# GenomicBreeding/GenomicBreedingModels.jl

Hardware: AMD Instinct MI355X
Metric: GRM+GBLUP genotype-cells/s (n x p) (higher is better)
Workload: dtype f64

## Files before the change

### genomicbreedingmodels.jl_amd/csrc/gbm_internal.h

```cpp
#pragma once
#include <hip/hip_runtime.h>
#include <stdint.h>
#include <functional>
#include <string>
#include <vector>

#include "../../include/gbm.h"

namespace gbm {

constexpr int64_t kNPadTile = 128;
constexpr int64_t kRhsRows = 64;
constexpr int kCholNB = 64;

inline int64_t round_up(int64_t x, int64_t m) { return (x + m - 1) / m * m; }
inline int64_t npad_of(int64_t n) { return round_up(n < 1 ? 1 : n, kNPadTile); }
inline int64_t gdim_of(int64_t n) { return npad_of(n) + kRhsRows; }

void set_error(const std::string& msg);
int fail(int code, const std::string& msg);
const std::string& last_error();

const char* knob(const char* name);
int64_t knob_i64(const char* name, int64_t def);

#define GBM_HIP_TRY(expr)                                                                      \
  do {                                                                                         \
    hipError_t e_ = (expr);                                                                    \
    if (e_ != hipSuccess)                                                                      \
      return ::gbm::fail(GBM_E_HIP, std::string("HIP error '") + hipGetErrorString(e_) +       \
                                        "' at " __FILE__ ":" + std::to_string(__LINE__) + " (" #expr ")"); \
  } while (0)

#define GBM_LAUNCH_CHECK() GBM_HIP_TRY(hipGetLastError())

#define GBM_TRY(expr)              \
  do {                             \
    int rc_ = (expr);              \
    if (rc_ != GBM_OK) return rc_; \
  } while (0)

int launch_grm(const double* Zt, int64_t ldz, int64_t p, int64_t n, double* G, int64_t ldg,
               void* ws, int64_t ws_bytes, hipStream_t s, int accum = 0, int32_t* err_out = nullptr);
bool grm_can_accumulate(int64_t n, int64_t p);
int64_t grm_workspace_bytes(int64_t n, int64_t p);
int launch_grm_export(const double* G, int64_t ldg, int64_t n, double inv_q, double* out, int64_t ldo, hipStream_t s);
int launch_predict(const double* Xt, int64_t ldx, int64_t p, int64_t n, const double* b, int64_t ldb, int64_t nrhs,
                   double* partial, int64_t nchunks, double* out, int64_t ldo, hipStream_t s);
int64_t predict_chunks(int64_t n, int64_t p);
int launch_add_inplace(double* a, const double* b, int64_t n, hipStream_t s);
int launch_standardize_i8(const int8_t* D, int64_t ldd, int64_t p, int64_t n, int ploidy, double* Zt, int64_t ldz,
                          double* mean, double* sd, int32_t* keep, int64_t* q_dev, hipStream_t s);
int launch_marker_rows(const double* Zt, int64_t ldz, int64_t p, int64_t n, const double* A, int64_t lda, int64_t nrhs,
                       double inv_q, const int64_t* q_dev, const double* sd, const int32_t* keep, double* B,
                       int64_t ldb, hipStream_t s);
int launch_marker_rows_i8(const int8_t* D, int64_t ldd, int64_t p, int64_t n, int ploidy, const double* A, int64_t lda,
                          int64_t nrhs, double inv_q, const int64_t* q_dev, const double* mean, const double* sd,
                          const int32_t* keep, double* B, int64_t ldb, hipStream_t s);
int launch_grm_exact(const int8_t* D, int64_t ldd, int64_t p, int64_t n, int ploidy, double* G, int64_t ldg,
                     double* mean, double* sd, int32_t* keep, int64_t* q_dev, int accum, void* ws, int64_t ws_bytes,
                     int32_t* slices_out, hipStream_t s);
int grm_exact_status(const void* ws, int64_t n, int64_t p, hipStream_t s);
int launch_gather_dosage(const double* Xt, int64_t ldx, int64_t p, const int32_t* idx, int64_t nT, int8_t* D,
                         hipStream_t s);
int launch_dosage_from_f64(const double* X, int64_t ldx, int64_t n, int64_t p, int8_t* D, int64_t ldd, int32_t* bad,
                           hipStream_t s);
int launch_dosage_check_i8(const int8_t* D, int64_t ldd, int64_t n, int64_t p, int32_t* bad, hipStream_t s);
// ... 58 lines not shown
```

### genomicbreedingmodels.jl_amd/csrc/grm.hip

```cpp
#include <algorithm>
#include <atomic>
#include <cmath>
#include <cstdio>
#include <cstdlib>
#include <map>
#include <mutex>
#include <queue>
#include <tuple>
#include <vector>

#include "chol_device.h"

namespace gbm {

constexpr int BT = 128;
constexpr int BK = 16;
constexpr int WPS = 2;
constexpr int LROW = BT + 2;
constexpr int STAGE = 2 * BK * LROW;

__device__ __forceinline__ void tile_of(int64_t t, int64_t& ti, int64_t& tj) {
  int64_t r = (int64_t)((sqrt(8.0 * (double)t + 1.0) - 1.0) * 0.5);
  while ((r + 1) * (r + 2) / 2 <= t) r++;
  while (r * (r + 1) / 2 > t) r--;
// ... 148 lines not shown

__device__ __forceinline__ void diag_tile(const double* __restrict__ U, int64_t ldu, int64_t K, int64_t i0,
                                          int64_t kstep0, int64_t nsteps, double* lds, double* __restrict__ out,
                                          int64_t ld, int wave, int lane) {
  asm volatile("" : "+v"(lane));
  switch (wave) {
    case 0: diag_tile_wave<0>(U, ldu, K, i0, kstep0, nsteps, lds, out, ld, lane); break;
    case 1: diag_tile_wave<1>(U, ldu, K, i0, kstep0, nsteps, lds, out, ld, lane); break;
    case 2: diag_tile_wave<2>(U, ldu, K, i0, kstep0, nsteps, lds, out, ld, lane); break;
    default: diag_tile_wave<3>(U, ldu, K, i0, kstep0, nsteps, lds, out, ld, lane); break;
  }
}

constexpr int kMaxSlices = 32;
struct SliceBounds {
  int32_t n;
  int32_t b[kMaxSlices + 1];
  int32_t carry;
  int32_t er, et, erb, es, ekper;
  int64_t e0, eslab_off;
  int32_t accum = 0;
  int32_t fuse = 0;
  int32_t diag = 0;
};

template <int ET>
__device__ __forceinline__ void grm_edge_pass(const double* __restrict__ U, int64_t ldu, int64_t K,
                                              const SliceBounds& sb, int64_t e, double* __restrict__ part,
                                              int lane, int wave) {
  const int rb = (int)(e % sb.erb), ks = (int)(e / sb.erb);
  const int64_t k0 = (int64_t)ks * sb.ekper;
  const int64_t k1 = (k0 + sb.ekper < K) ? k0 + sb.ekper : K;
  const int64_t i0 = (int64_t)rb * 256 + wave * 64;
  const int fr = lane >> 4, fc = lane & 15;
  d4 acc[4][ET];
#pragma unroll
  for (int m = 0; m < 4; m++)
#pragma unroll
    for (int q = 0; q < ET; q++) acc[m][q] = (d4){0.0, 0.0, 0.0, 0.0};
  for (int64_t k = k0; k < k1; k += 16) {
    double a[4][4], b[4][ET];
#pragma unroll
    for (int st = 0; st < 4; st++) {
      const int64_t kk = k + st * 4 + fr;
      const bool kv = kk < k1;
      const double* row = U + kk * ldu;
// ... 189 lines not shown
#pragma unroll
        for (int r = 0; r < 4; r++) {
          double* o = out + (16 * r + m) * ld;
          *reinterpret_cast<double2*>(o) = make_double2(acc[m][0][r], acc[m][1][r]);
          *reinterpret_cast<double2*>(o + 2) = make_double2(acc[m][2][r], acc[m][3][r]);
        }
    }
    };
    const int64_t T8 = (ntiles + 7) & ~(int64_t)7;
    if constexpr (MODE == kPersist || MODE == kPersistFused) {
      __shared__ int64_t s_unit;
      int32_t* ctr = info;
      const int xcc = (int)(__builtin_amdgcn_s_getreg((20 << 0) | (0 << 6) | (31 << 11)) & 7);
      const int64_t per = T8 >> 3;
      int q = xcc;
      for (int tries = 0; tries < 8;) {
        const int64_t qt0 = q * per;
        const int64_t qt1 = qt0 + per < ntiles ? qt0 + per : ntiles;
        const int64_t nq = qt1 > qt0 ? qt1 - qt0 : 0;
        if (threadIdx.x == 0) s_unit = atomicAdd(&ctr[q], 1);
        __syncthreads();
        const int64_t u = s_unit;
        __syncthreads();
        if (u >= nq * sb.n) {
          q = (q + 1) & 7;
          tries++;
          continue;
        }
        const int sl = (int)(u / nq);
        run_unit(sl, qt0 + (u - (int64_t)sl * nq));
      }
      return;
    } else {
      const int sl = (int)(wg / T8);
      const int64_t u = wg - (int64_t)sl * T8;
      const int64_t t = (u & 7) * (T8 >> 3) + (u >> 3);
      if (t >= ntiles) return;
      run_unit(sl, t);
    }
    return;
  } else {
    int64_t ti, tj;
    if (own.nranks > 1) {
      const int64_t c = blockIdx.y;
      const int64_t J = c < own.ncols ? own.j_first + c * own.nranks : own.rhs_tile;
      tj = J - c0 / BT;
      ti = own.ti0 + blockIdx.x;
      if (ti > tj) return;
    } else {
      tile_of(wg, ti, tj);
    }
    const bool diag = (ti == tj);
    const int64_t i0 = c0 + ti * BT, j0 = c0 + tj * BT;
// ... 464 lines not shown
  GBM_HIP_TRY(hipGetDevice(&dev));
  if (caller) {
    int sdev = -1;
    if (hipStreamGetDevice(caller, &sdev) != hipSuccess) {
      (void)hipGetLastError();
      return GBM_OK;
    }
    if (sdev != dev) return GBM_OK;
  }
  static std::mutex mu;
  static std::map<int, hipStream_t> streams;
  {
    std::lock_guard<std::mutex> lock(mu);
    hipStream_t& hs = streams[dev];
    if (!hs) GBM_HIP_TRY(hipStreamCreateWithFlags(&hs, hipStreamNonBlocking));
    a.s = hs;
  }
  GBM_HIP_TRY(hipEventCreateWithFlags(&a.fork, hipEventDisableTiming));
  GBM_HIP_TRY(hipEventCreateWithFlags(&a.join, hipEventDisableTiming));
  *usable = true;
  return GBM_OK;
}

static int64_t grm_counter_doubles(const GrmPlan& g) { return 4 + (g.sb.fuse ? (g.ntiles + 1) / 2 : 0); }
int64_t grm_workspace_bytes(int64_t n, int64_t p) {
  const GrmPlan g = plan(n, p);
  return (g.main_doubles + g.edge_doubles + grm_counter_doubles(g)) * (int64_t)sizeof(double);
}

static int check_grm_args(const double* Zt, int64_t ldz, int64_t p, int64_t n, double* G, int64_t ldg) {
  const int64_t npad = npad_of(n);
  if (!Zt || !G || p < 1 || n < 1 || ldz < npad || ldg < npad || (ldz & 1) || (ldg & 1))
    return fail(GBM_E_ARG, "gbm_dev_grm: bad arguments (need ldz, ldg >= npad(n), both even)");
  if (((uintptr_t)Zt & 15) != 0 || ((uintptr_t)G & 15) != 0)
    return fail(GBM_E_ARG, "gbm_dev_grm: Zt and G must be 16-byte aligned");
  return GBM_OK;
}

int launch_grm_syrk(const double* Zt, int64_t ldz, int64_t p, int64_t n, double* G, int64_t ldg, void* ws,
                    int64_t ws_bytes, hipStream_t s, int accum = 0) {
  int rc = check_grm_args(Zt, ldz, p, n, G, ldg);
  if (rc != GBM_OK) return rc;
  const GrmPlan g = plan(n, p);
  SliceBounds sb = g.sb;
  sb.accum = accum;
  const int64_t need = (g.main_doubles + g.edge_doubles + grm_counter_doubles(g)) * (int64_t)sizeof(double);
  if (need > 0 && (!ws || ws_bytes < need))
    return fail(GBM_E_ARG, "gbm_dev_grm: workspace too small (" + std::to_string(ws_bytes) + " < " +
                               std::to_string(need) + ")");
  const unsigned grid = (unsigned)(g.sb.n * ((g.ntiles + 7) & ~(int64_t)7));
  if (g.sb.carry) GBM_HIP_TRY(hipMemsetAsync(ws, 0, (size_t)(g.ntiles + 1) * sizeof(int32_t), s));
  int32_t* ctr = reinterpret_cast<int32_t*>((double*)ws + g.main_doubles + g.edge_doubles);
  const int64_t lim = g.sb.er > 0 ? g.sb.e0 : n;
  AuxStream aux;
  AuxStream* ax = nullptr;
  if (g.edge_concurrent) {
    bool usable = false;
    rc = aux_stream(s, aux, &usable);
    if (rc != GBM_OK) return rc;
    if (usable) {
      ax = &aux;
      GBM_HIP_TRY(hipEventRecord(ax->fork, s));
      GBM_HIP_TRY(hipStreamWaitEvent(ax->s, ax->fork, 0));
    }
  }
  if (g.persist) {
    GBM_HIP_TRY(hipMemsetAsync(ctr, 0, (size_t)(8 + (g.sb.fuse ? g.ntiles : 0)) * sizeof(int32_t), s));
    const int64_t units = (int64_t)g.sb.n * g.ntiles;
    const unsigned pgrid = (unsigned)(units < resident_wgs() ? units : resident_wgs());
    if (g.sb.fuse)
      syrk_kernel<kPersistFused><<<pgrid, 256, 0, s>>>(Zt, ldz, p, 0, lim, G, ldg, (double*)ws, g.ntiles, sb, nullptr,
                                                       nullptr, ctr, -1, TileOwner{});
    else
      syrk_kernel<kPersist><<<pgrid, 256, 0, s>>>(Zt, ldz, p, 0, lim, G, ldg, (double*)ws, g.ntiles, sb, nullptr,
                                                  nullptr, ctr, -1, TileOwner{});
  } else {
    syrk_kernel<kSplit><<<grid, 256, 0, s>>>(Zt, ldz, p, 0, lim, G, ldg, (double*)ws, g.ntiles, sb, nullptr, nullptr,
                                             nullptr, -1, TileOwner{});
  }
  GBM_LAUNCH_CHECK();
  if (g.sb.er > 0) {
    const hipStream_t es = ax ? ax->s : s;
    const unsigned eg = (unsigned)((int64_t)g.sb.erb * g.sb.es);
    double* part = (double*)ws + g.sb.eslab_off;
    switch (g.sb.et) {
      case 1: grm_edge_kernel<1><<<eg, 256, 0, es>>>(Zt, ldz, p, g.sb, part); break;
      case 2: grm_edge_kernel<2><<<eg, 256, 0, es>>>(Zt, ldz, p, g.sb, part); break;
      case 3: grm_edge_kernel<3><<<eg, 256, 0, es>>>(Zt, ldz, p, g.sb, part); break;
      default: grm_edge_kernel<4><<<eg, 256, 0, es>>>(Zt, ldz, p, g.sb, part); break;
    }
    GBM_LAUNCH_CHECK();
    if (g.edge_concurrent) {
      grm_edge_reduce_kernel<<<(unsigned)((n * g.sb.er + 255) / 256), 256, 0, es>>>(part, n, g.sb, G, ldg, accum);
      GBM_LAUNCH_CHECK();
    }
    if (ax) {
      GBM_HIP_TRY(hipEventRecord(ax->join, ax->s));
      GBM_HIP_TRY(hipStreamWaitEvent(s, ax->join, 0));
    }
  }
  return GBM_OK;
}

int launch_grm_reduce(int64_t n, int64_t p, double* G, int64_t ldg, const void* ws, hipStream_t s, int accum = 0,
                      int32_t* err_out = nullptr) {
  const GrmPlan g = plan(n, p);
  if (g.sb.n == 1 && g.sb.er == 0) return GBM_OK;
  if (!ws) return fail(GBM_E_ARG, "gbm_dev_grm_reduce: workspace required");
  if (g.sb.er > 0 && !g.edge_concurrent) {
    grm_edge_reduce_kernel<<<(unsigned)((n * g.sb.er + 255) / 256), 256, 0, s>>>((const double*)ws + g.sb.eslab_off, n,
                                                                                 g.sb, G, ldg, accum);
    GBM_LAUNCH_CHECK();
  }
  if (g.sb.n == 1 || g.sb.fuse) return GBM_OK;
  if (g.sb.carry && err_out) {
    GBM_HIP_TRY(hipMemcpyAsync(err_out, (const int32_t*)ws + g.ntiles, sizeof(int32_t), hipMemcpyDeviceToDevice, s));
    return GBM_OK;
  }
  if (g.sb.carry) {
    int32_t err = 0;
    GBM_HIP_TRY(hipMemcpyAsync(&err, (const int32_t*)ws + g.ntiles, sizeof(int32_t), hipMemcpyDeviceToHost, s));
    GBM_HIP_TRY(hipStreamSynchronize(s));
    if (err < 0)
// ... 59 lines not shown
  return GBM_OK;
}

extern "C" int64_t gbm_dev_grm_workspace(int64_t n, int64_t p) { return gbm::grm_workspace_bytes(n, p); }

extern "C" int gbm_dev_grm(const double* Zt, int64_t ldz, int64_t p, int64_t n, double* G, int64_t ldg,
                           void* workspace, int64_t ws_bytes, void* stream) {
  return gbm::launch_grm(Zt, ldz, p, n, G, ldg, workspace, ws_bytes, (hipStream_t)stream);
}

extern "C" int gbm_dev_grm_accumulate(const double* Zt, int64_t ldz, int64_t p, int64_t n, double* G, int64_t ldg,
                                      void* workspace, int64_t ws_bytes, void* stream) {
  if (!gbm::grm_can_accumulate(n, p))
    return gbm::fail(GBM_E_ARG, "gbm_dev_grm_accumulate: this (n, p) plans a single loci range (gbm_dev_grm_slices == 1); "
                                "use more loci per call");
  return gbm::launch_grm(Zt, ldz, p, n, G, ldg, workspace, ws_bytes, (hipStream_t)stream, 1);
}

extern "C" int gbm_dev_grm_syrk(const double* Zt, int64_t ldz, int64_t p, int64_t n, double* G, int64_t ldg,
                                void* workspace, int64_t ws_bytes, void* stream) {
  return gbm::launch_grm_syrk(Zt, ldz, p, n, G, ldg, workspace, ws_bytes, (hipStream_t)stream);
}

extern "C" int gbm_dev_grm_reduce(int64_t n, int64_t p, double* G, int64_t ldg, const void* workspace, void* stream) {
  if (!G || n < 1 || p < 1 || ldg < gbm::npad_of(n)) return gbm::fail(GBM_E_ARG, "gbm_dev_grm_reduce: bad arguments");
  return gbm::launch_grm_reduce(n, p, G, ldg, workspace, (hipStream_t)stream);
}

extern "C" int gbm_dev_grm_slices(int64_t n, int64_t p) {
  return gbm::plan(n, p).sb.n;
}

namespace gbm {
__global__ void __launch_bounds__(256) add_inplace_kernel(double* __restrict__ a, const double* __restrict__ b,
                                                          int64_t n) {
  for (int64_t i = ((int64_t)blockIdx.x * 256 + threadIdx.x) * 2; i < n; i += (int64_t)gridDim.x * 512) {
    if (i + 1 < n) {
      double2 x = *reinterpret_cast<const double2*>(a + i);
      const double2 y = *reinterpret_cast<const double2*>(b + i);
      x.x += y.x;
      x.y += y.y;
      *reinterpret_cast<double2*>(a + i) = x;
    } else {
      a[i] += b[i];
    }
  }
// ... 24 lines not shown
```

### genomicbreedingmodels.jl_amd/csrc/stats.hip

```cpp
#include <type_traits>

#include "gbm_internal.h"

namespace gbm {

__device__ __forceinline__ uint64_t mix64(uint64_t z) {
  z += 0x9E3779B97F4A7C15ull;
  z = (z ^ (z >> 30)) * 0xBF58476D1CE4E5B9ull;
  z = (z ^ (z >> 27)) * 0x94D049BB133111EBull;
  return z ^ (z >> 31);
}

__global__ void __launch_bounds__(256) synth_kernel(double* __restrict__ Xt, int64_t ldx, int64_t p,
                                                    int64_t n, uint64_t seed, int64_t j0) {
  for (int64_t j = blockIdx.y; j < p; j += gridDim.y) {
    const uint64_t base = mix64(seed * 0xD1B54A32D192ED03ull + (uint64_t)(j0 + j));
    const uint64_t thr = 214748364ull + (((base >> 32) * 1932735283ull) >> 32);
    double* row = Xt + j * ldx;
    for (int64_t i = (int64_t)blockIdx.x * 1024 + threadIdx.x; i < (int64_t)(blockIdx.x + 1) * 1024 && i < ldx;
         i += 256) {
      double v = 0.0;
      if (i < n) {
        const uint64_t h = mix64(base ^ ((uint64_t)i * 0x8CB92BA72F3D8DD7ull));
        const int d = ((h & 0xFFFFFFFFull) < thr) + ((h >> 32) < thr);
// ... 251 lines not shown
    else if (n <= 64 * 64) GBM_STD_W(64);
    else if (n <= 64 * 80) GBM_STD_W(80);
    else if (n <= 64 * 96) GBM_STD_W(96);
    else GBM_STD_W(128);
#undef GBM_STD_W
    GBM_LAUNCH_CHECK();
    return GBM_OK;
  }
  if (n <= 256 * 4)
    standardize_kernel<256, 4, GATHER, T><<<grid, 256, 0, s>>>(Xt, ldx, p, idx, n, Zt, ldz, mean, sd, keep, q, center_only, xs);
  else if (n <= 256 * 8)
    standardize_kernel<256, 8, GATHER, T><<<grid, 256, 0, s>>>(Xt, ldx, p, idx, n, Zt, ldz, mean, sd, keep, q, center_only, xs);
  else if (n <= 256 * 16)
    standardize_kernel<256, 16, GATHER, T><<<grid, 256, 0, s>>>(Xt, ldx, p, idx, n, Zt, ldz, mean, sd, keep, q, center_only, xs);
  else if (n <= 256 * 32)
    standardize_kernel<256, 32, GATHER, T><<<grid, 256, 0, s>>>(Xt, ldx, p, idx, n, Zt, ldz, mean, sd, keep, q, center_only, xs);
  else
    standardize_kernel<256, 0, GATHER, T><<<grid, 256, 0, s>>>(Xt, ldx, p, idx, n, Zt, ldz, mean, sd, keep, q, center_only, xs);
  GBM_LAUNCH_CHECK();
  return GBM_OK;
}

namespace gbm {
int launch_center_columns(const double* Xt, int64_t ldx, int64_t p, int64_t n, double* Zt, int64_t ldz, double* mean,
                          double* sd, int32_t* keep, int64_t* q_dev, hipStream_t s) {
  if (p == 0) return GBM_OK;
  return launch_standardize<false>(Xt, ldx, p, nullptr, n, Zt, ldz, mean, sd, keep, q_dev, 1, s);
}

int launch_standardize_i8(const int8_t* D, int64_t ldd, int64_t p, int64_t n, int ploidy, double* Zt, int64_t ldz,
                          double* mean, double* sd, int32_t* keep, int64_t* q_dev, hipStream_t s) {
  if (!D || !Zt || !mean || !sd || !keep || !q_dev || p < 0 || n < 1 || ldd < n || ldz < n || ploidy < 1)
    return fail(GBM_E_ARG, "standardize (int8 dosages): bad arguments");
  if (p == 0) return GBM_OK;
  return launch_standardize<false, int8_t>(D, ldd, p, nullptr, n, Zt, ldz, mean, sd, keep, q_dev, 0, s, 1.0 / ploidy);
}
}

extern "C" int gbm_dev_standardize(const double* Xt, int64_t ldx, int64_t p, int64_t n, double* Zt, int64_t ldz,
                                   double* mean, double* sd, int32_t* keep, int64_t* q_dev, void* stream) {
  if (!Xt || !Zt || !mean || !sd || !keep || !q_dev || p < 0 || n < 1 || ldx < n || ldz < n ||
      ((const double*)Zt == Xt && ldz != ldx))
    return fail(GBM_E_ARG, "gbm_dev_standardize: bad arguments");
  if (p == 0) return GBM_OK;
  return launch_standardize<false>(Xt, ldx, p, nullptr, n, Zt, ldz, mean, sd, keep, q_dev, 0, (hipStream_t)stream);
}
// ... 18 lines not shown
```

### genomicbreedingmodels.jl_amd/gbm/_lib.py

```python
from __future__ import annotations

import ctypes
import os
import threading

import numpy as np

ABI_VERSION = 212
GBM_OK = 0
GBM_E_ARG = -1
GBM_E_NOTPD = -2
GBM_E_HIP = -3
GBM_E_RCCL = -4
GBM_E_OOM = -5
GBM_E_NODEV = -6
GBM_E_DATA = -7

LIB_PATH = os.environ.get("GBM_LIBGBM") or os.path.join(os.path.dirname(os.path.abspath(__file__)), "libgbm.so")

EXPORTS = (
    "gbm_version", "gbm_last_error", "gbm_device_count", "gbm_device_allocations", "gbm_release_device_cache",
    "gbm_gblup_fit", "gbm_gblup_fit_reml", "gbm_gblup_fit_dosage_i8", "gbm_gblup_fit_synthetic", "gbm_grm", "gbm_grm_ploidy_aware", "gbm_colstats", "gbm_predict",
    "gbm_dev_npad", "gbm_dev_gdim", "gbm_dev_grm_workspace", "gbm_dev_solve_workspace",
    "gbm_dev_synth_genotypes", "gbm_dev_expand_dosage_i8", "gbm_dev_standardize", "gbm_dev_grm",
    "gbm_dev_grm_syrk", "gbm_dev_grm_reduce", "gbm_dev_grm_slices",
    "gbm_dev_gblup_solve", "gbm_dev_marker_effects",
    "gbm_dev_standardize_gather", "gbm_dev_gblup_terms",
    "gbm_session_create", "gbm_session_create_dosage_i8", "gbm_session_create_synthetic", "gbm_session_destroy", "gbm_session_gblup_fit",
    "gbm_session_predict", "gbm_session_reml_objective", "gbm_session_reml", "gbm_session_stats",
    "gbm_session_ridge_path", "gbm_session_ridge_lambda_max", "gbm_brr_fit", "gbm_bayes_fit",
    "gbm_dev_chol_prepare", "gbm_dev_chol_prepare_cols", "gbm_dev_chol_group_size", "gbm_dev_chol_group", "gbm_dev_chol_factor_diag",
    "gbm_dev_chol_strip_doubles", "gbm_dev_chol_strip_pack", "gbm_dev_chol_strip_unpack", "gbm_dev_chol_finish",
    "gbm_dev_grm_packed_size", "gbm_dev_grm_pack", "gbm_dev_grm_unpack",
    "gbm_debug_brr_stats", "gbm_debug_brr_shape", "gbm_debug_brr_trace", "gbm_debug_chol_flow_trace",
    "gbm_dev_synth_dosage_i8", "gbm_dev_standardize_i8", "gbm_dev_grm_accumulate", "gbm_dev_marker_effects_i8",
    "gbm_debug_oom_retries", "gbm_dev_chol_group_panels", "gbm_dev_chol_group_update", "gbm_dev_chol_strip_unpack_rows", "gbm_dev_chol_lower_copy",
    "gbm_dev_chol_area_doubles", "gbm_dev_chol_area_pack", "gbm_dev_chol_area_unpack",
    "gbm_dev_chol_group_update_cols", "gbm_dev_chol_group_update_tiles", "gbm_dev_grm_exact_workspace", "gbm_dev_grm_exact_i8",
    "gbm_gblup_fit_ex", "gbm_gblup_fit_reml_ex", "gbm_gblup_fit_dosage_i8_ex", "gbm_gblup_fit_synthetic_ex",
    "gbm_session_set_grm_mode", "gbm_session_grm_used", "gbm_debug_rccl_calls", "gbm_debug_xg_choose", "gbm_debug_chol_flow_order",
    "gbm_debug_chol_flow_order_check", "gbm_debug_chol_flow_order_size", "gbm_dev_grm_exact_status", "gbm_debug_set",
    "gbm_dev_whiten_rows", "gbm_session_gwas", "gbm_session_enet_path",
)

GBM_GRM_DEFAULT, GBM_GRM_FP64, GBM_GRM_EXACT, GBM_GRM_AUTO, GBM_GRM_DROPIN = -1, 0, 1, 2, 3
GRM_MODES = {None: GBM_GRM_DEFAULT, "default": GBM_GRM_DEFAULT, "fp64": GBM_GRM_FP64, "exact": GBM_GRM_EXACT,
             "auto": GBM_GRM_AUTO, "dropin": GBM_GRM_DROPIN}


def grm_mode(mode) -> int:
    if isinstance(mode, int) and mode in GRM_MODES.values():
        return mode
    try:
        return GRM_MODES[mode]
    except (KeyError, TypeError):
        raise ArgumentError(f"grm must be one of 'auto', 'exact', 'fp64', 'dropin' or None, got {mode!r}") from None


class ArgumentError(ValueError):
    """Mirrors Julia's ArgumentError thrown by the reference (e.g. src/prediction.jl:67-112)."""


class GBMError(RuntimeError):
    """Mirrors Julia's ErrorException (e.g. src/linear.jl:235-237, src/prediction.jl:125-127)."""

# ... 75 lines not shown
        getattr(lib, f).argtypes = [I64]
    for f in ("gbm_dev_grm_workspace", "gbm_dev_solve_workspace"):
        getattr(lib, f).restype = I64
        getattr(lib, f).argtypes = [I64, I64]
    lib.gbm_dev_synth_genotypes.restype = I32
    lib.gbm_dev_synth_genotypes.argtypes = [P, I64, I64, I64, U64, I64, P]
    lib.gbm_dev_expand_dosage_i8.restype = I32
    lib.gbm_dev_expand_dosage_i8.argtypes = [P, I64, I64, I64, I32, P, I64, P]
    lib.gbm_dev_standardize.restype = I32
    lib.gbm_dev_standardize.argtypes = [P, I64, I64, I64, P, I64, P, P, P, P, P]
    lib.gbm_dev_synth_dosage_i8.restype = I32
    lib.gbm_dev_synth_dosage_i8.argtypes = [P, I64, I64, I64, U64, I64, P]
    lib.gbm_dev_standardize_i8.restype = I32
    lib.gbm_dev_standardize_i8.argtypes = [P, I64, I64, I64, I32, P, I64, P, P, P, P, P]
    lib.gbm_dev_marker_effects_i8.restype = I32
    lib.gbm_dev_grm_exact_workspace.restype = I64
    lib.gbm_dev_grm_exact_workspace.argtypes = [I64, I64]
    lib.gbm_dev_grm_exact_i8.restype = I32
    lib.gbm_dev_grm_exact_i8.argtypes = [P, I64, I64, I64, I32, P, I64, P, P, P, P, I32, P, I64, P, P]
    lib.gbm_dev_marker_effects_i8.argtypes = [P, I64, I64, I64, I32, P, I64, I64, D, P, P, P, P, P, I64, P, P]
    for f in ("gbm_dev_grm", "gbm_dev_grm_syrk", "gbm_dev_grm_accumulate"):
        getattr(lib, f).restype = I32
        getattr(lib, f).argtypes = [P, I64, I64, I64, P, I64, P, I64, P]
    lib.gbm_dev_grm_reduce.restype = I32
    lib.gbm_dev_grm_reduce.argtypes = [I64, I64, P, I64, P, P]
    lib.gbm_dev_grm_slices.restype = I32
    lib.gbm_dev_grm_slices.argtypes = [I64, I64]
    lib.gbm_dev_gblup_solve.restype = I32
    lib.gbm_dev_gblup_solve.argtypes = [P, I64, I64, D, P, D, P, I64, I64, P, P, I64, P, P, P, I64, P]
    lib.gbm_dev_marker_effects.restype = I32
    lib.gbm_dev_marker_effects.argtypes = [P, I64, I64, I64, P, I64, I64, D, P, P, P, P, P, I64, P, P]
    lib.gbm_dev_standardize_gather.restype = I32
    lib.gbm_dev_standardize_gather.argtypes = [P, I64, I64, P, I64, P, I64, P, P, P, P, I32, P]
    lib.gbm_dev_gblup_terms.restype = I32
    lib.gbm_dev_gblup_terms.argtypes = [P, I64, I64, I64, P, P, P]
    lib.gbm_session_create.restype = I32
    lib.gbm_session_create.argtypes = [P, I64, I64, I64, I32, ctypes.POINTER(P)]
    lib.gbm_session_create_synthetic.restype = I32
    lib.gbm_session_create_synthetic.argtypes = [U64, I64, I64, I32, ctypes.POINTER(P)]
    lib.gbm_session_create_dosage_i8.restype = I32
    lib.gbm_session_create_dosage_i8.argtypes = [P, I64, I64, I64, I32, I32, ctypes.POINTER(P)]
    lib.gbm_session_destroy.restype = None
    lib.gbm_session_destroy.argtypes = [P]
    lib.gbm_session_gblup_fit.restype = I32
    lib.gbm_session_gblup_fit.argtypes = [P, P, I64, P, I64, I64, D, P, P, P, P]
    lib.gbm_session_predict.restype = I32
# ... 120 lines not shown
```

### genomicbreedingmodels.jl_amd/gbm/sharded.py

```python
from __future__ import annotations

import ctypes

import numpy as np

from . import _lib


class TorchComm:

    def __init__(self, force: bool = False):
        import torch.distributed as dist
        self.dist = dist
        self.world_size = dist.get_world_size() if dist.is_initialized() else 1
        self.rank = dist.get_rank() if dist.is_initialized() else 0
        self.force = bool(force) and dist.is_initialized()

    def all_reduce_sum(self, t):
        if self.world_size > 1 or self.force:
            self.dist.all_reduce(t, op=self.dist.ReduceOp.SUM)

    def all_gather(self, t):
        import torch
        out = torch.empty(self.world_size * t.numel(), dtype=t.dtype, device=t.device)
# ... 175 lines not shown
        kb = k1
        if kb >= nb:
            break
        dist = next_dist
        if not dist:
            exchange(kb, nb - kb, "rest")
    for st in stages:
        if defer_lower:
            st.lower_join()
        st.chol_finish()


def assemble_b_hat(mu, msum, B_shards, p_total):
    t = len(mu)
    b_hat = np.zeros((p_total + 1, t))
    b_hat[0] = np.asarray(mu) - np.asarray(msum)
    off = 0
    for B in B_shards:
        b_hat[1 + off:1 + off + B.shape[1]] = B.T
        off += B.shape[1]
    return b_hat


class HipShardStages:

    def __init__(self, n: int, p_local: int, nrhs: int = 1, lambda_: float = 1.0, device: int = 0):
        import torch
        self.torch = torch
        self.lib = _lib.load()
        self.n, self.p, self.nrhs, self.lam = n, p_local, nrhs, float(lambda_)
        self.dev = torch.device("cuda", device)
        lib = self.lib
        self.npad = lib.gbm_dev_npad(n)
        self.gdim = lib.gbm_dev_gdim(n)
        f64 = dict(dtype=torch.float64, device=self.dev)
        self._alloc_rows(f64)
        self.mean = torch.empty(p_local, **f64)
        self.sd = torch.empty(p_local, **f64)
        self.keep = torch.empty(p_local, dtype=torch.int32, device=self.dev)
        self.q = torch.zeros(1, dtype=torch.int64, device=self.dev)
        self.G = torch.empty((self.gdim, self.gdim), **f64)
        self.ws_grm_bytes = self._grm_workspace()
        self.ws_grm = torch.empty(max(self.ws_grm_bytes, 16), dtype=torch.uint8, device=self.dev)
        self.Y = torch.zeros((nrhs, self.npad), **f64)
        self.A = torch.zeros((nrhs, self.npad), **f64)
        self.ws_solve_bytes = lib.gbm_dev_solve_workspace(n, nrhs)
# ... 21 lines not shown
    @staticmethod
    def _p(t):
        return ctypes.c_void_p(t.data_ptr())

    def _stream(self):
        return ctypes.c_void_p(self.torch.cuda.current_stream(self.dev).cuda_stream)

    def generate(self, seed: int, j0: int):
        _lib.check(self.lib.gbm_dev_synth_genotypes(self._p(self.X), self.npad, self.p, self.n, seed, j0,
                                                     self._stream()), "synth")

    def upload_genotypes(self, X_host_colmajor: np.ndarray):
        t = self.torch.from_numpy(np.ascontiguousarray(np.asarray(X_host_colmajor, dtype=np.float64).T))
        self.X.zero_()
        self.X[:, :self.n].copy_(t)

    def load_phenotypes(self, Y: np.ndarray):
        Y = np.asarray(Y, dtype=np.float64)
        if Y.ndim == 1:
            Y = Y[:, None]
        self.Y.zero_()
        self.Y[:, :self.n].copy_(self.torch.from_numpy(np.ascontiguousarray(Y.T)))

    def standardize(self):
        self.q.zero_()
        _lib.check(self.lib.gbm_dev_standardize(self._p(self.X), self.npad, self.p, self.n, self._p(self.Z), self.npad,
                                                self._p(self.mean), self._p(self.sd), self._p(self.keep),
                                                self._p(self.q), self._stream()), "standardize")

    def grm_syrk(self):
        _lib.check(self.lib.gbm_dev_grm_syrk(self._p(self.Z), self.npad, self.p, self.n, self._p(self.G), self.gdim,
                                             self._p(self.ws_grm), self.ws_grm_bytes, self._stream()), "grm_syrk")

    def grm_reduce(self):
        _lib.check(self.lib.gbm_dev_grm_reduce(self.n, self.p, self._p(self.G), self.gdim, self._p(self.ws_grm),
                                               self._stream()), "grm_reduce")

    def grm_rows(self):
        return self.G[: self.npad]

    def grm_pack(self):
        if getattr(self, "Gp", None) is None:
            self.Gp = self.torch.empty(self.lib.gbm_dev_grm_packed_size(self.n) + 1, dtype=self.torch.float64,
                                       device=self.dev)
        _lib.check(self.lib.gbm_dev_grm_pack(self._p(self.G), self.gdim, self.n, self._p(self.Gp), self._stream()),
                   "grm_pack")
        self.Gp[-1:].copy_(self.q)
        return self.Gp

    def grm_unpack(self):
        _lib.check(self.lib.gbm_dev_grm_unpack(self._p(self.Gp), self.n, self._p(self.G), self.gdim, self._stream()),
                   "grm_unpack")
        self.q.copy_(self.Gp[-1:])
# ... 244 lines not shown
```

### include/gbm.h

```cpp
#ifndef GBM_H
#define GBM_H

#include <stdint.h>

#ifdef __cplusplus
extern "C" {
#endif

#define GBM_VERSION 212

#define GBM_OK 0
#define GBM_E_ARG (-1)
#define GBM_E_NOTPD (-2)
#define GBM_E_HIP (-3)
#define GBM_E_RCCL (-4)
#define GBM_E_OOM (-5)
#define GBM_E_NODEV (-6)
#define GBM_E_DATA (-7)

#define GBM_GRM_DEFAULT (-1)
#define GBM_GRM_FP64 0
#define GBM_GRM_EXACT 1
#define GBM_GRM_AUTO 2
#define GBM_GRM_DROPIN 3
// ... 73 lines not shown
                            int64_t j0, void* stream);

int gbm_dev_synth_dosage_i8(int8_t* D, int64_t ldd, int64_t p, int64_t n, uint64_t seed, int64_t j0,
                            void* stream);

int gbm_dev_expand_dosage_i8(const int8_t* D, int64_t ldd, int64_t n, int64_t p, int ploidy,
                             double* Xt, int64_t ldx, void* stream);

int gbm_dev_standardize(const double* Xt, int64_t ldx, int64_t p, int64_t n, double* Zt, int64_t ldz,
                        double* mean, double* sd, int32_t* keep, int64_t* q_dev, void* stream);
int gbm_dev_standardize_i8(const int8_t* D, int64_t ldd, int64_t p, int64_t n, int ploidy, double* Zt, int64_t ldz,
                           double* mean, double* sd, int32_t* keep, int64_t* q_dev, void* stream);
int gbm_dev_standardize_gather(const double* Xt, int64_t ldx, int64_t p, const int32_t* idx, int64_t n,
                               double* Zt, int64_t ldz, double* mean, double* sd, int32_t* keep,
                               int64_t* q_dev, int center_only, void* stream);

int gbm_dev_grm(const double* Zt, int64_t ldz, int64_t p, int64_t n, double* G, int64_t ldg,
                void* workspace, int64_t ws_bytes, void* stream);
int gbm_dev_grm_accumulate(const double* Zt, int64_t ldz, int64_t p, int64_t n, double* G, int64_t ldg,
                           void* workspace, int64_t ws_bytes, void* stream);
int gbm_dev_grm_syrk(const double* Zt, int64_t ldz, int64_t p, int64_t n, double* G, int64_t ldg,
                     void* workspace, int64_t ws_bytes, void* stream);
int gbm_dev_grm_reduce(int64_t n, int64_t p, double* G, int64_t ldg, const void* workspace, void* stream);
int64_t gbm_dev_grm_packed_size(int64_t n);
int gbm_dev_grm_pack(const double* G, int64_t ldg, int64_t n, double* packed, void* stream);
int gbm_dev_grm_unpack(const double* packed, int64_t n, double* G, int64_t ldg, void* stream);
int gbm_dev_grm_slices(int64_t n, int64_t p);

int gbm_dev_gblup_solve(double* G, int64_t ldg, int64_t n, double inv_q, const int64_t* q_dev, double lambda,
                        const double* Y, int64_t ldy, int64_t nrhs,
                        double* A_out, double* gebv, int64_t lda, double* mu, int32_t* info,
                        void* workspace, int64_t ws_bytes, void* stream);

int gbm_dev_chol_prepare(double* G, int64_t ldg, int64_t n, double inv_q, const int64_t* q_dev, double lambda,
                         const double* Y, int64_t ldy, int64_t nrhs, int32_t* info, void* workspace,
                         int64_t ws_bytes, void* stream);
int gbm_dev_chol_prepare_cols(double* G, int64_t ldg, int64_t n, double inv_q, const int64_t* q_dev, double lambda,
                              const double* Y, int64_t ldy, int64_t nrhs, int rank, int nranks, int32_t* info,
                              void* workspace, int64_t ws_bytes, void* stream);
int64_t gbm_dev_chol_group_size(int64_t n, int64_t kb);
int gbm_dev_chol_group(double* G, int64_t ldg, int64_t n, int64_t kb, int rank, int nranks, int32_t* info,
                       void* workspace, int64_t ws_bytes, void* stream);
int gbm_dev_chol_group_panels(double* G, int64_t ldg, int64_t n, int64_t kb, int rank, int nranks, int32_t* info,
                              void* workspace, int64_t ws_bytes, void* stream);
int gbm_dev_chol_group_update(double* G, int64_t ldg, int64_t n, int64_t kb, int rank, int nranks, int32_t* info,
                              void* workspace, int64_t ws_bytes, void* stream);
// ... 111 lines not shown
```

Baseline: 11.97 billion.

## Overlap marker standardization with first GRM slice on an auxiliary stream

Adds a fused standardize+GRM entry point. It standardizes only the first slice of markers, launches the persistent SYRK for slice 0, and meanwhile standardizes the remaining markers on an auxiliary stream before running the other slices there. The Python stage object defers standardize() lazily so grm_syrk can take the fused path. The cost targeted is the serial dependency between standardization and the GRM kernel. The trade-offs are extra workspace for a second counter block, cross-stream contention for compute units, and more complex lazy-property state.

```diff
diff --git a/genomicbreedingmodels.jl_amd/csrc/gbm_internal.h b/genomicbreedingmodels.jl_amd/csrc/gbm_internal.h
--- a/genomicbreedingmodels.jl_amd/csrc/gbm_internal.h
+++ b/genomicbreedingmodels.jl_amd/csrc/gbm_internal.h
@@ -43,6 +43,9 @@
 int launch_grm(const double* Zt, int64_t ldz, int64_t p, int64_t n, double* G, int64_t ldg,
                void* ws, int64_t ws_bytes, hipStream_t s, int accum = 0, int32_t* err_out = nullptr);
 bool grm_can_accumulate(int64_t n, int64_t p);
+int launch_standardize_rows(const double* Xt, int64_t ldx, int64_t p, int64_t n, double* Zt, int64_t ldz, double* mean,
+                            double* sd, int32_t* keep, int64_t* q_dev, hipStream_t s, bool beside_tiles = false);
+bool standardize_fits_beside_tiles(int64_t n);
 int64_t grm_workspace_bytes(int64_t n, int64_t p);
 int launch_grm_export(const double* G, int64_t ldg, int64_t n, double inv_q, double* out, int64_t ldo, hipStream_t s);
 int launch_predict(const double* Xt, int64_t ldx, int64_t p, int64_t n, const double* b, int64_t ldb, int64_t nrhs,
diff --git a/genomicbreedingmodels.jl_amd/csrc/grm.hip b/genomicbreedingmodels.jl_amd/csrc/grm.hip
--- a/genomicbreedingmodels.jl_amd/csrc/grm.hip
+++ b/genomicbreedingmodels.jl_amd/csrc/grm.hip
@@ -194,6 +194,7 @@
   int32_t accum = 0;
   int32_t fuse = 0;
   int32_t diag = 0;
+  int32_t s0 = 0, cnt = 0;
 };
 
 template <int ET>
@@ -429,13 +430,13 @@
         __syncthreads();
         const int64_t u = s_unit;
         __syncthreads();
-        if (u >= nq * sb.n) {
+        if (u >= nq * sb.cnt) {
           q = (q + 1) & 7;
           tries++;
           continue;
         }
-        const int sl = (int)(u / nq);
-        run_unit(sl, qt0 + (u - (int64_t)sl * nq));
+        const int r = (int)(u / nq);
+        run_unit(sb.s0 + r, qt0 + (u - (int64_t)r * nq));
       }
       return;
     } else {
@@ -946,7 +947,12 @@
   return GBM_OK;
 }
 
-static int64_t grm_counter_doubles(const GrmPlan& g) { return 4 + (g.sb.fuse ? (g.ntiles + 1) / 2 : 0); }
+static int64_t grm_second_doubles(const GrmPlan& g) {
+  return (g.persist && !g.sb.fuse && g.sb.n >= 2) ? g.tile_elems : 0;
+}
+static int64_t grm_counter_doubles(const GrmPlan& g) {
+  return grm_second_doubles(g) + 4 + (g.sb.fuse ? (g.ntiles + 1) / 2 : 0);
+}
 int64_t grm_workspace_bytes(int64_t n, int64_t p) {
   const GrmPlan g = plan(n, p);
   return (g.main_doubles + g.edge_doubles + grm_counter_doubles(g)) * (int64_t)sizeof(double);
@@ -958,6 +964,40 @@
     return fail(GBM_E_ARG, "gbm_dev_grm: bad arguments (need ldz, ldg >= npad(n), both even)");
   if (((uintptr_t)Zt & 15) != 0 || ((uintptr_t)G & 15) != 0)
     return fail(GBM_E_ARG, "gbm_dev_grm: Zt and G must be 16-byte aligned");
+  return GBM_OK;
+}
+
+static int launch_persist(const GrmPlan& g, SliceBounds sb, int s0, int cnt, const double* Zt, int64_t ldz, int64_t p,
+                          int64_t lim, double* G, int64_t ldg, void* ws, int32_t* ctr, hipStream_t s) {
+  sb.s0 = s0;
+  sb.cnt = cnt;
+  const int64_t units = (int64_t)cnt * g.ntiles;
+  const unsigned pgrid = (unsigned)(units < resident_wgs() ? units : resident_wgs());
+  if (g.sb.fuse)
+    syrk_kernel<kPersistFused><<<pgrid, 256, 0, s>>>(Zt, ldz, p, 0, lim, G, ldg, (double*)ws, g.ntiles, sb, nullptr,
+                                                     nullptr, ctr, -1, TileOwner{});
+  else
+    syrk_kernel<kPersist><<<pgrid, 256, 0, s>>>(Zt, ldz, p, 0, lim, G, ldg, (double*)ws, g.ntiles, sb, nullptr,
+                                                nullptr, ctr, -1, TileOwner{});
+  GBM_LAUNCH_CHECK();
+  return GBM_OK;
+}
+
+static int launch_grm_edge(const GrmPlan& g, const double* Zt, int64_t ldz, int64_t p, int64_t n, double* G,
+                           int64_t ldg, void* ws, int accum, hipStream_t es) {
+  const unsigned eg = (unsigned)((int64_t)g.sb.erb * g.sb.es);
+  double* part = (double*)ws + g.sb.eslab_off;
+  switch (g.sb.et) {
+    case 1: grm_edge_kernel<1><<<eg, 256, 0, es>>>(Zt, ldz, p, g.sb, part); break;
+    case 2: grm_edge_kernel<2><<<eg, 256, 0, es>>>(Zt, ldz, p, g.sb, part); break;
+    case 3: grm_edge_kernel<3><<<eg, 256, 0, es>>>(Zt, ldz, p, g.sb, part); break;
+    default: grm_edge_kernel<4><<<eg, 256, 0, es>>>(Zt, ldz, p, g.sb, part); break;
+  }
+  GBM_LAUNCH_CHECK();
+  if (g.edge_concurrent) {
+    grm_edge_reduce_kernel<<<(unsigned)((n * g.sb.er + 255) / 256), 256, 0, es>>>(part, n, g.sb, G, ldg, accum);
+    GBM_LAUNCH_CHECK();
+  }
   return GBM_OK;
 }
 
@@ -974,7 +1014,7 @@
                                std::to_string(need) + ")");
   const unsigned grid = (unsigned)(g.sb.n * ((g.ntiles + 7) & ~(int64_t)7));
   if (g.sb.carry) GBM_HIP_TRY(hipMemsetAsync(ws, 0, (size_t)(g.ntiles + 1) * sizeof(int32_t), s));
-  int32_t* ctr = reinterpret_cast<int32_t*>((double*)ws + g.main_doubles + g.edge_doubles);
+  int32_t* ctr = reinterpret_cast<int32_t*>((double*)ws + g.main_doubles + g.edge_doubles + grm_second_doubles(g));
   const int64_t lim = g.sb.er > 0 ? g.sb.e0 : n;
   AuxStream aux;
   AuxStream* ax = nullptr;
@@ -990,39 +1030,62 @@
   }
   if (g.persist) {
     GBM_HIP_TRY(hipMemsetAsync(ctr, 0, (size_t)(8 + (g.sb.fuse ? g.ntiles : 0)) * sizeof(int32_t), s));
-    const int64_t units = (int64_t)g.sb.n * g.ntiles;
-    const unsigned pgrid = (unsigned)(units < resident_wgs() ? units : resident_wgs());
-    if (g.sb.fuse)
-      syrk_kernel<kPersistFused><<<pgrid, 256, 0, s>>>(Zt, ldz, p, 0, lim, G, ldg, (double*)ws, g.ntiles, sb, nullptr,
-                                                       nullptr, ctr, -1, TileOwner{});
-    else
-      syrk_kernel<kPersist><<<pgrid, 256, 0, s>>>(Zt, ldz, p, 0, lim, G, ldg, (double*)ws, g.ntiles, sb, nullptr,
-                                                  nullptr, ctr, -1, TileOwner{});
+    rc = launch_persist(g, sb, 0, g.sb.n, Zt, ldz, p, lim, G, ldg, ws, ctr, s);
+    if (rc != GBM_OK) return rc;
   } else {
     syrk_kernel<kSplit><<<grid, 256, 0, s>>>(Zt, ldz, p, 0, lim, G, ldg, (double*)ws, g.ntiles, sb, nullptr, nullptr,
                                              nullptr, -1, TileOwner{});
-  }
-  GBM_LAUNCH_CHECK();
+    GBM_LAUNCH_CHECK();
+  }
   if (g.sb.er > 0) {
-    const hipStream_t es = ax ? ax->s : s;
-    const unsigned eg = (unsigned)((int64_t)g.sb.erb * g.sb.es);
-    double* part = (double*)ws + g.sb.eslab_off;
-    switch (g.sb.et) {
-      case 1: grm_edge_kernel<1><<<eg, 256, 0, es>>>(Zt, ldz, p, g.sb, part); break;
-      case 2: grm_edge_kernel<2><<<eg, 256, 0, es>>>(Zt, ldz, p, g.sb, part); break;
-      case 3: grm_edge_kernel<3><<<eg, 256, 0, es>>>(Zt, ldz, p, g.sb, part); break;
-      default: grm_edge_kernel<4><<<eg, 256, 0, es>>>(Zt, ldz, p, g.sb, part); break;
-    }
-    GBM_LAUNCH_CHECK();
-    if (g.edge_concurrent) {
-      grm_edge_reduce_kernel<<<(unsigned)((n * g.sb.er + 255) / 256), 256, 0, es>>>(part, n, g.sb, G, ldg, accum);
-      GBM_LAUNCH_CHECK();
-    }
+    rc = launch_grm_edge(g, Zt, ldz, p, n, G, ldg, ws, accum, ax ? ax->s : s);
+    if (rc != GBM_OK) return rc;
     if (ax) {
       GBM_HIP_TRY(hipEventRecord(ax->join, ax->s));
       GBM_HIP_TRY(hipStreamWaitEvent(s, ax->join, 0));
     }
   }
+  return GBM_OK;
+}
+
+int launch_standardize_grm_syrk(const double* X, int64_t ldx, int64_t p, int64_t n, double* Zt, int64_t ldz,
+                                double* mean, double* sd, int32_t* keep, int64_t* q, double* G, int64_t ldg, void* ws,
+                                int64_t ws_bytes, hipStream_t s) {
+  int rc = check_grm_args(Zt, ldz, p, n, G, ldg);
+  if (rc != GBM_OK) return rc;
+  if (!X || !mean || !sd || !keep || !q || ldx < n || (X == Zt && ldx != ldz))
+    return fail(GBM_E_ARG, "gbm_dev_standardize_grm_syrk: bad arguments");
+  const GrmPlan g = plan(n, p);
+  const int64_t h = g.sb.n >= 2 ? std::min<int64_t>(p, (int64_t)BK * g.sb.b[1]) : p;
+  AuxStream aux;
+  bool overlap = knob_i64("GBM_GRM_STD_OVERLAP", 1) != 0 && g.persist && !g.sb.fuse && g.sb.n >= 2 && h < p &&
+                 standardize_fits_beside_tiles(n);
+  if (overlap) {
+    rc = aux_stream(s, aux, &overlap);
+    if (rc != GBM_OK) return rc;
+  }
+  if (!overlap) {
+    rc = launch_standardize_rows(X, ldx, p, n, Zt, ldz, mean, sd, keep, q, s);
+    if (rc != GBM_OK) return rc;
+    return launch_grm_syrk(Zt, ldz, p, n, G, ldg, ws, ws_bytes, s);
+  }
+  const int64_t need = (g.main_doubles + g.edge_doubles + grm_counter_doubles(g)) * (int64_t)sizeof(double);
+  if (!ws || ws_bytes < need)
+    return fail(GBM_E_ARG, "gbm_dev_standardize_grm_syrk: workspace too small (" + std::to_string(ws_bytes) + " < " +
+                               std::to_string(need) + ")");
+  int32_t* ctr = reinterpret_cast<int32_t*>((double*)ws + g.main_doubles + g.edge_doubles + grm_second_doubles(g)) - 8;
+  const int64_t lim = g.sb.er > 0 ? g.sb.e0 : n;
+  GBM_TRY(launch_standardize_rows(X, ldx, h, n, Zt, ldz, mean, sd, keep, q, s));
+  GBM_HIP_TRY(hipMemsetAsync(ctr, 0, 16 * sizeof(int32_t), s));
+  GBM_HIP_TRY(hipEventRecord(aux.fork, s));
+  GBM_HIP_TRY(hipStreamWaitEvent(aux.s, aux.fork, 0));
+  GBM_TRY(launch_persist(g, g.sb, 0, 1, Zt, ldz, p, lim, G, ldg, ws, ctr + 8, s));
+  GBM_TRY(launch_standardize_rows(X + h * ldx, ldx, p - h, n, Zt + h * ldz, ldz, mean + h, sd + h, keep + h, q, aux.s,
+                                  true));
+  if (g.sb.er > 0) GBM_TRY(launch_grm_edge(g, Zt, ldz, p, n, G, ldg, ws, 0, aux.s));
+  GBM_TRY(launch_persist(g, g.sb, 1, g.sb.n - 1, Zt, ldz, p, lim, G, ldg, ws, ctr, aux.s));
+  GBM_HIP_TRY(hipEventRecord(aux.join, aux.s));
+  GBM_HIP_TRY(hipStreamWaitEvent(s, aux.join, 0));
   return GBM_OK;
 }
 
@@ -1128,6 +1191,13 @@
   return gbm::launch_grm_syrk(Zt, ldz, p, n, G, ldg, workspace, ws_bytes, (hipStream_t)stream);
 }
 
+extern "C" int gbm_dev_standardize_grm_syrk(const double* Xt, int64_t ldx, int64_t p, int64_t n, double* Zt, int64_t ldz,
+                                            double* mean, double* sd, int32_t* keep, int64_t* q_dev, double* G,
+                                            int64_t ldg, void* workspace, int64_t ws_bytes, void* stream) {
+  return gbm::launch_standardize_grm_syrk(Xt, ldx, p, n, Zt, ldz, mean, sd, keep, q_dev, G, ldg, workspace, ws_bytes,
+                                          (hipStream_t)stream);
+}
+
 extern "C" int gbm_dev_grm_reduce(int64_t n, int64_t p, double* G, int64_t ldg, const void* workspace, void* stream) {
   if (!G || n < 1 || p < 1 || ldg < gbm::npad_of(n)) return gbm::fail(GBM_E_ARG, "gbm_dev_grm_reduce: bad arguments");
   return gbm::launch_grm_reduce(n, p, G, ldg, workspace, (hipStream_t)stream);
diff --git a/genomicbreedingmodels.jl_amd/csrc/stats.hip b/genomicbreedingmodels.jl_amd/csrc/stats.hip
--- a/genomicbreedingmodels.jl_amd/csrc/stats.hip
+++ b/genomicbreedingmodels.jl_amd/csrc/stats.hip
@@ -297,6 +297,20 @@
 }
 
 namespace gbm {
+bool standardize_fits_beside_tiles(int64_t n) { return n <= 256 * 20; }
+
+int launch_standardize_rows(const double* Xt, int64_t ldx, int64_t p, int64_t n, double* Zt, int64_t ldz, double* mean,
+                            double* sd, int32_t* keep, int64_t* q_dev, hipStream_t s, bool beside_tiles) {
+  if (p == 0) return GBM_OK;
+  if (beside_tiles && n > 256 * 16 && n <= 256 * 20) {
+    standardize_kernel<256, 20, false, double><<<(unsigned)(p < 256 * 16 ? p : 256 * 16), 256, 0, s>>>(
+        Xt, ldx, p, nullptr, n, Zt, ldz, mean, sd, keep, reinterpret_cast<unsigned long long*>(q_dev), 0, 1.0);
+    GBM_LAUNCH_CHECK();
+    return GBM_OK;
+  }
+  return launch_standardize<false>(Xt, ldx, p, nullptr, n, Zt, ldz, mean, sd, keep, q_dev, 0, s);
+}
+
 int launch_center_columns(const double* Xt, int64_t ldx, int64_t p, int64_t n, double* Zt, int64_t ldz, double* mean,
                           double* sd, int32_t* keep, int64_t* q_dev, hipStream_t s) {
   if (p == 0) return GBM_OK;
diff --git a/genomicbreedingmodels.jl_amd/gbm/_lib.py b/genomicbreedingmodels.jl_amd/gbm/_lib.py
--- a/genomicbreedingmodels.jl_amd/gbm/_lib.py
+++ b/genomicbreedingmodels.jl_amd/gbm/_lib.py
@@ -40,7 +40,7 @@
     "gbm_gblup_fit_ex", "gbm_gblup_fit_reml_ex", "gbm_gblup_fit_dosage_i8_ex", "gbm_gblup_fit_synthetic_ex",
     "gbm_session_set_grm_mode", "gbm_session_grm_used", "gbm_debug_rccl_calls", "gbm_debug_xg_choose", "gbm_debug_chol_flow_order",
     "gbm_debug_chol_flow_order_check", "gbm_debug_chol_flow_order_size", "gbm_dev_grm_exact_status", "gbm_debug_set",
-    "gbm_dev_whiten_rows", "gbm_session_gwas", "gbm_session_enet_path",
+    "gbm_dev_whiten_rows", "gbm_session_gwas", "gbm_session_enet_path", "gbm_dev_standardize_grm_syrk",
 )
 
 GBM_GRM_DEFAULT, GBM_GRM_FP64, GBM_GRM_EXACT, GBM_GRM_AUTO, GBM_GRM_DROPIN = -1, 0, 1, 2, 3
@@ -162,6 +162,8 @@
     for f in ("gbm_dev_grm", "gbm_dev_grm_syrk", "gbm_dev_grm_accumulate"):
         getattr(lib, f).restype = I32
         getattr(lib, f).argtypes = [P, I64, I64, I64, P, I64, P, I64, P]
+    lib.gbm_dev_standardize_grm_syrk.restype = I32
+    lib.gbm_dev_standardize_grm_syrk.argtypes = [P, I64, I64, I64, P, I64, P, P, P, P, P, I64, P, I64, P]
     lib.gbm_dev_grm_reduce.restype = I32
     lib.gbm_dev_grm_reduce.argtypes = [I64, I64, P, I64, P, P]
     lib.gbm_dev_grm_slices.restype = I32
diff --git a/genomicbreedingmodels.jl_amd/gbm/sharded.py b/genomicbreedingmodels.jl_amd/gbm/sharded.py
--- a/genomicbreedingmodels.jl_amd/gbm/sharded.py
+++ b/genomicbreedingmodels.jl_amd/gbm/sharded.py
@@ -221,6 +221,20 @@
     return b_hat
 
 
+def _written_by_standardize(name):
+    attr = "_" + name
+
+    def get(self):
+        if self._std_pending:
+            self._standardize_now()
+        return getattr(self, attr)
+
+    def put(self, value):
+        setattr(self, attr, value)
+
+    return property(get, put)
+
+
 class HipShardStages:
 
     def __init__(self, n: int, p_local: int, nrhs: int = 1, lambda_: float = 1.0, device: int = 0):
@@ -288,13 +302,31 @@
         self.Y.zero_()
         self.Y[:, :self.n].copy_(self.torch.from_numpy(np.ascontiguousarray(Y.T)))
 
+    _std_pending = False
+    Z = _written_by_standardize("Z")
+    mean = _written_by_standardize("mean")
+    sd = _written_by_standardize("sd")
+    keep = _written_by_standardize("keep")
+    q = _written_by_standardize("q")
+
     def standardize(self):
-        self.q.zero_()
-        _lib.check(self.lib.gbm_dev_standardize(self._p(self.X), self.npad, self.p, self.n, self._p(self.Z), self.npad,
-                                                self._p(self.mean), self._p(self.sd), self._p(self.keep),
-                                                self._p(self.q), self._stream()), "standardize")
+        self._q.zero_()
+        self._std_pending = True
+
+    def _standardize_now(self):
+        self._std_pending = False
+        _lib.check(self.lib.gbm_dev_standardize(self._p(self.X), self.npad, self.p, self.n, self._p(self._Z), self.npad,
+                                                self._p(self._mean), self._p(self._sd), self._p(self._keep),
+                                                self._p(self._q), self._stream()), "standardize")
 
     def grm_syrk(self):
+        if self._std_pending:
+            self._std_pending = False
+            _lib.check(self.lib.gbm_dev_standardize_grm_syrk(
+                self._p(self.X), self.npad, self.p, self.n, self._p(self._Z), self.npad, self._p(self._mean),
+                self._p(self._sd), self._p(self._keep), self._p(self._q), self._p(self.G), self.gdim,
+                self._p(self.ws_grm), self.ws_grm_bytes, self._stream()), "standardize_grm_syrk")
+            return
         _lib.check(self.lib.gbm_dev_grm_syrk(self._p(self.Z), self.npad, self.p, self.n, self._p(self.G), self.gdim,
                                              self._p(self.ws_grm), self.ws_grm_bytes, self._stream()), "grm_syrk")
 
diff --git a/include/gbm.h b/include/gbm.h
--- a/include/gbm.h
+++ b/include/gbm.h
@@ -119,6 +119,9 @@
 int gbm_dev_grm_syrk(const double* Zt, int64_t ldz, int64_t p, int64_t n, double* G, int64_t ldg,
                      void* workspace, int64_t ws_bytes, void* stream);
 int gbm_dev_grm_reduce(int64_t n, int64_t p, double* G, int64_t ldg, const void* workspace, void* stream);
+int gbm_dev_standardize_grm_syrk(const double* Xt, int64_t ldx, int64_t p, int64_t n, double* Zt, int64_t ldz,
+                                 double* mean, double* sd, int32_t* keep, int64_t* q_dev, double* G, int64_t ldg,
+                                 void* workspace, int64_t ws_bytes, void* stream);
 int64_t gbm_dev_grm_packed_size(int64_t n);
 int gbm_dev_grm_pack(const double* G, int64_t ldg, int64_t n, double* packed, void* stream);
 int gbm_dev_grm_unpack(const double* packed, int64_t n, double* G, int64_t ldg, void* stream);
```

Result: faster. 12.11 billion (median of 6 runs) (+1.2%).
